# ratt-ru/pfb-clean

Hardware: AMD Instinct MI355X
Metric: PCG matvecs/sec (FFT-conv A^H A apply), 4k x 4k x 8-band cube (higher is better)
Workload: dtype f32; 1 GPU; 4096x4096x8-band cube PCG (hessian_psf + Tikhonov, M = x/sigmainv, tol=0, minit=maxit=20); nx_psf=8192, bands_per_gpu=8, parallelism=band-shard x1, allreduce_hook=False

## Files before the change

### include/pfb_hip.h

```cpp
#ifndef PFB_HIP_H
#define PFB_HIP_H

#include <stddef.h>
#include <stdint.h>

#ifdef __cplusplus
extern "C" {
#endif

#define PFB_ABI_VERSION 1

#define PFB_F32 0
#define PFB_F64 1

#define PFB_OK               0
#define PFB_ERR_INVALID     -1
#define PFB_ERR_UNSUPPORTED -2
#define PFB_ERR_HIP         -3
#define PFB_ERR_NONFINITE   -4
#define PFB_ERR_ALLOC       -5
#define PFB_ERR_COMM        -6

#define PFB_PCG_CONVERGED     0
#define PFB_PCG_MAXIT         1
#define PFB_PCG_ZERO_RESIDUAL 2
#define PFB_PCG_BREAKDOWN     3

int         pfb_abi_version(void);
const char* pfb_last_error(void);

typedef struct pfb_conv_plan pfb_conv_plan;

int pfb_psfconv_plan_create(int nx, int ny, int nx_psf, int ny_psf, int nband,
                            int dtype, pfb_conv_plan** plan);
int pfb_psfconv_plan_destroy(pfb_conv_plan* plan);

int pfb_psfconv_set_psfhat(pfb_conv_plan* plan, const void* psfhat, void* stream);

int pfb_psfconv_set_psf(pfb_conv_plan* plan, const void* psf, void* psfhat_out, void* stream);

int pfb_psfhat_from_psf(int dtype, const void* psf, int nband, int nx_psf, int ny_psf, void* psfhat, void* stream);

int pfb_psfhat_regrid(int dtype, const void* psfhat, int nband, int nx, int ny, int nx_psf, int ny_psf,
                      int nx_psf2, int ny_psf2, void* psfhat2, void* stream);

int pfb_psfconv_apply(pfb_conv_plan* plan, int band0, int nb,
                      const void* x, const void* beam, double wsum, double sigmainv,
                      void* out, const void* dot_with, double* dot_out, void* stream);

int pfb_psfconv_apply_dots(pfb_conv_plan* plan, int band0, int nb,
                           const void* x, const void* beam, double wsum, double sigmainv,
                           void* out, const void* dot_with, const void* dot_with2,
                           double* dots_out, void* stream);

int    pfb_psfconv_plan_info(const pfb_conv_plan* plan, int* fast_path, int* vb,
                             size_t* workspace_bytes);

int pfb_psfconv_set_profiling(pfb_conv_plan* plan, int on);
int pfb_psfconv_get_profile(pfb_conv_plan* plan, double stage_ms[3], int* napply);

#define PFB_REDUCE_WS_DOUBLES 8192

int pfb_dot(int dtype, const void* a, const void* b, size_t n,
            double* out, double* ws, void* stream);
int pfb_norm_diff_sums(int dtype, const void* x, const void* xp, size_t n,
                       double* out, double* ws, void* stream);
int pfb_any_nonzero(int dtype, const void* a, size_t n, double* out, double* ws,
                    void* stream);
int pfb_axpby(int dtype, double a, const void* x, double b, void* y, size_t n,
              void* stream);

typedef int (*pfb_allreduce_fn)(void* ctx, double* dev_buf, int count, void* stream);

typedef struct {
    int    status;
    int    iters;
    int    matvecs;
    int    backtracks;
    double eps;
    double rnorm;
} pfb_pcg_result;

size_t pfb_pcg_work_bytes(const pfb_conv_plan* plan, int nb);
int pfb_pcg_solve(pfb_conv_plan* plan, int band0, int nb,
                  const void* b, void* x, void* r_out,
                  const void* beam, double wsum, double sigmainv, double mdiv,
                  double tol, int maxit, int minit, int backtrack,
                  void* work, pfb_allreduce_fn allreduce, void* allreduce_ctx,
                  pfb_pcg_result* result, void* stream);
// ... 65 lines not shown
```

### pfb_clean_amd/_lib.py

```python
import ctypes as C
import os

_HERE = os.path.dirname(os.path.abspath(__file__))
LIB_PATH = os.environ.get('PFB_HIP_LIB') or os.path.join(_HERE, 'libpfb_hip.so')

PFB_F32, PFB_F64 = 0, 1
PFB_OK = 0
ERRORS = {-1: 'invalid argument', -2: 'unsupported size/dtype', -3: 'HIP runtime error',
          -4: 'non-finite value', -5: 'device allocation failed', -6: 'band-shard exchange failed'}
PCG_STATUS = {0: 'converged', 1: 'maxit', 2: 'zero-residual', 3: 'breakdown'}
REDUCE_WS_DOUBLES = 8192


PFB_ERR_INVALID = -1
PFB_ERR_UNSUPPORTED = -2
PFB_ERR_ALLOC = -5
PFB_ERR_COMM = -6


class PfbHipError(RuntimeError):
    def __init__(self, code, msg):
        super().__init__(f"libpfb_hip: {ERRORS.get(code, code)}: {msg}")
        self.code = code


class PfbCommError(PfbHipError):
    """PFB_ERR_COMM: the band-shard exchange of a distributed solve failed, was aborted or timed out.  The exchange has
    been torn down; this rank holds no result and should exit non-zero (its peers get the same error)."""


class PcgResult(C.Structure):
    _fields_ = [('status', C.c_int), ('iters', C.c_int), ('matvecs', C.c_int),
                ('backtracks', C.c_int), ('eps', C.c_double), ('rnorm', C.c_double)]


ALLREDUCE_FN = C.CFUNCTYPE(C.c_int, C.c_void_p, C.c_void_p, C.c_int, C.c_void_p)

_vp, _i, _d, _sz = C.c_void_p, C.c_int, C.c_double, C.c_size_t
SIGNATURES = {
    'pfb_abi_version': (_i, []),
    'pfb_last_error': (C.c_char_p, []),
    'pfb_psfconv_plan_create': (_i, [_i, _i, _i, _i, _i, _i, C.POINTER(_vp)]),
    'pfb_psfconv_plan_destroy': (_i, [_vp]),
    'pfb_psfconv_set_psfhat': (_i, [_vp, _vp, _vp]),
    'pfb_psfconv_apply': (_i, [_vp, _i, _i, _vp, _vp, _d, _d, _vp, _vp, _vp, _vp]),
    'pfb_psfconv_set_psf': (_i, [_vp, _vp, _vp, _vp]),
    'pfb_psfhat_regrid': (_i, [_i, _vp, _i, _i, _i, _i, _i, _i, _i, _vp, _vp]),
    'pfb_psfhat_from_psf': (_i, [_i, _vp, _i, _i, _i, _vp, _vp]),
    'pfb_psfconv_apply_dots': (_i, [_vp, _i, _i, _vp, _vp, _d, _d, _vp, _vp, _vp, _vp, _vp]),
    'pfb_psfconv_plan_info': (_i, [_vp, C.POINTER(_i), C.POINTER(_i), C.POINTER(_sz)]),
    'pfb_psfconv_set_profiling': (_i, [_vp, _i]),
    'pfb_psfconv_get_profile': (_i, [_vp, C.POINTER(_d), C.POINTER(_i)]),
    'pfb_dot': (_i, [_i, _vp, _vp, _sz, _vp, _vp, _vp]),
    'pfb_norm_diff_sums': (_i, [_i, _vp, _vp, _sz, _vp, _vp, _vp]),
    'pfb_any_nonzero': (_i, [_i, _vp, _sz, _vp, _vp, _vp]),
    'pfb_axpby': (_i, [_i, _d, _vp, _d, _vp, _sz, _vp]),
    'pfb_pcg_work_bytes': (_sz, [_vp, _i]),
    'pfb_pcg_solve': (_i, [_vp, _i, _i, _vp, _vp, _vp, _vp, _d, _d, _d, _d, _i, _i, _i,
                           _vp, ALLREDUCE_FN, _vp, C.POINTER(PcgResult), _vp]),
    'pfb_comm_bind': (_i, [C.c_char_p]),
    'pfb_comm_unique_id': (_i, [_vp]),
    'pfb_comm_init': (_i, [_i, _i, _vp, C.POINTER(_vp)]),
    'pfb_comm_destroy': (_i, [_vp]),
    'pfb_comm_info': (_i, [_vp, C.POINTER(_i), C.POINTER(_i), C.POINTER(_i), C.POINTER(_i)]),
    'pfb_comm_allreduce': (_i, [_vp, _vp, _i, _vp]),
    'pfb_comm_check': (_i, [_vp]),
    'pfb_comm_abort': (_i, [_vp]),
    'pfb_psi_plan_create': (_i, [_i, _i, _i, _i, C.POINTER(_i), C.POINTER(_d), _i, _i,
                                 C.POINTER(_vp)]),
    'pfb_psi_plan_destroy': (_i, [_vp]),
    'pfb_psi_plan_dims': (_i, [_vp, C.POINTER(_i), C.POINTER(_i)]),
    'pfb_psi_dot': (_i, [_vp, _vp, _vp, _vp]),
    'pfb_psi_hdot': (_i, [_vp, _vp, _vp, _vp]),
    'pfb_dual_update': (_i, [_i, _vp, _vp, _vp, _d, _d, _i, _sz, _vp, _vp]),
    'pfb_dual_bandsum': (_i, [_i, _vp, _vp, _d, _i, _sz, _vp, _vp]),
    'pfb_dual_apply': (_i, [_i, _vp, _vp, _vp, _vp, _d, _d, _i, _sz, _vp, _vp]),
    'pfb_prox_21': (_i, [_i, _vp, _vp, _vp, _d, _d, _i, _sz, _vp]),
    'pfb_dual_update_l2': (_i, [_i, _vp, _vp, _vp, _d, _d, _i, _sz, _vp]),
    'pfb_dual_bandsum_chunk': (_i, [_i, _vp, _vp, _d, _i, _sz, _sz, _vp, _vp]),
    'pfb_dual_apply_chunk': (_i, [_i, _vp, _vp, _vp, _vp, _d, _d, _i, _sz, _sz, _vp, _vp]),
    'pfb_clark_subminor': (_i, [_i, _vp, _sz, _i, _vp, _i, _i, _vp, _vp, _vp, _i, _i, _vp, _d, _d, _i, _vp, _vp]),
    'pfb_hogbom': (_i, [_i, _vp, _vp, _vp, _vp, _i, _i, _i, _i, _i, _d, _d, _d, _i, _vp, _sz, _vp, _vp, _vp]),
    'pfb_freqmul': (_i, [_i, _vp, _vp, _vp, _i, _sz, _vp, _vp, _vp]),
# ... 32 lines not shown
```

### pfb_clean_amd/csrc/cgvec.hip

```cpp
#include "conv_plan.hpp"
#include "pcg_state.hpp"
#include <chrono>
#include <unistd.h>
#include <cstring>
#include <cstdlib>

namespace pfb {

constexpr int RED_BLOCK = 256;
constexpr int RED_MAX_GRID = 1024;

static inline int red_grid(size_t nvec) {
    size_t g = (nvec + RED_BLOCK - 1) / RED_BLOCK;
    g = (g + 3) / 4;
    if (g < 1) g = 1;
    if (g > (size_t)RED_MAX_GRID) g = RED_MAX_GRID;
    return (int)g;
}

template <typename T> struct V16;
template <> struct V16<float>  { using type = float4;  static constexpr int N = 4; };
template <> struct V16<double> { using type = double2; static constexpr int N = 2; };

template <typename T, int V> struct Pack { T e[V]; };
// ... 523 lines not shown
    err = pfb_psfconv_apply(plan, band0, nb, xcur, beam, wsum, sigmainv, rcur, nullptr, nullptr, (void*)st);
    if (err != PFB_OK) return err;
    res->matvecs = 1;
    PFB_LAUNCH_VEC(T, k_pcg_init, n, (PL{rcur, b, p}), rcur, (const T*)b, p, mdiv);
    hipLaunchKernelGGL(k_final_sum, dim3(1), dim3(RED_BLOCK), 0, st, ws, G_used, 2, S + S_RHON);
    if ((err = reduce_hook(S_RHON, 2)) != PFB_OK) return err;
    hipLaunchKernelGGL(k_init_state, dim3(1), dim3(1), 0, st, S, tol, (double)minit, (double)maxit);
    if ((err = fetch()) != PFB_OK) return err;
    if (h[S_NUM] == 0.0) {
        res->status = PFB_PCG_ZERO_RESIDUAL;
        res->eps = 1.0;
        res->rnorm = h[S_RHO];
        if (r_out) PFB_HIP_CHECK(hipMemcpyAsync(r_out, rcur, n * sizeof(T), hipMemcpyDeviceToDevice, st));
        return wait_stream();
    }

    int k = 0;
    double eps = 1.0;
    double rho = h[S_RHO];
    int status = -1;
    if (backtrack != 1) {
        int khost = 0;
        bool pending_end = false;
        bool go = (1.0 > tol || 0 < minit) && 0 < maxit;
        bool lookahead = n <= ((size_t)4 << 20);
        if (const char* la = getenv("PFB_PCG_LOOKAHEAD")) lookahead = atoi(la) != 0;
        if (lookahead && !plan->pcg_pin) {
            PFB_HIP_CHECK(hipHostMalloc((void**)&plan->pcg_pin, sizeof(double) * 2 * S_NSCALAR, hipHostMallocDefault));
            PFB_HIP_CHECK(hipEventCreateWithFlags(&plan->pcg_ev[0], hipEventDisableTiming));
            PFB_HIP_CHECK(hipEventCreateWithFlags(&plan->pcg_ev[1], hipEventDisableTiming));
        }
        int slot = 0;
        bool have_prev = false, stale_h = false;
        while (go) {
            err = psfconv_apply_partials(plan, band0, nb, p, beam, wsum, sigmainv, Ap, p, rcur, (void*)st);
            if (err != PFB_OK) return err;
            const int predict = backtrack == 2 ? 2 : 3;
            hipLaunchKernelGGL(k_iter_sums, dim3(1), dim3(256), 0, st, (const double*)plan->partials,
                               plan->last_npartials, (const double*)ws, G_used, pending_end ? 1 : 0, S,
                               mdiv_d, predict, allreduce ? 0 : 1);
            if (allreduce) {
                if ((err = reduce_hook(S_PAP, pending_end ? 7 : 4)) != PFB_OK) return err;
                if (pending_end)
                    hipLaunchKernelGGL(k_iter_end_begin, dim3(1), dim3(1), 0, st, S, mdiv_d, predict);
                else
                    hipLaunchKernelGGL(k_iter_begin, dim3(1), dim3(1), 0, st, S, mdiv_d, predict);
            }
            pending_end = false;
            G_used = launch_update_dir<T>(n, xcur, rcur, p, Ap, xnew, rnew, S + S_ALPHA, mdiv, ws, st);
            if (khost + 1 < minit && khost + 1 < maxit) {
                pending_end = true;
            } else if (!allreduce) {
                hipLaunchKernelGGL(k_final_sum_waves_end, dim3(1), dim3(256), 0, st, ws, G_used, S);
            } else {
                hipLaunchKernelGGL(k_final_sum_waves, dim3(1), dim3(256), 0, st, ws, G_used, 4, S,
                                   (Dst4{{S_RHON, S_NUM, S_DEN, S_ANY}}));
                if ((err = reduce_hook(S_RHON, 3)) != PFB_OK) return err;
                hipLaunchKernelGGL(k_iter_end, dim3(1), dim3(1), 0, st, S, 1);
            }
            { T* t = xcur; xcur = xnew; xnew = t; t = rcur; rcur = rnew; rnew = t; }
            ++khost;
            if (khost < minit && khost < maxit) continue;
            if (lookahead && khost < maxit) {
                double* snap = plan->pcg_pin + (size_t)slot * S_NSCALAR;
                PFB_HIP_CHECK(hipMemcpyAsync(snap, S, sizeof(double) * S_NSCALAR, hipMemcpyDeviceToHost, st));
                PFB_HIP_CHECK(hipEventRecord(plan->pcg_ev[slot], st));
                stale_h = true;
                if (have_prev) {
                    if (allreduce) {
                        const auto t0 = std::chrono::steady_clock::now();
                        for (long spins = 0;; ++spins) {
                            const hipError_t q = hipEventQuery(plan->pcg_ev[slot ^ 1]);
                            if (q == hipSuccess) break;
                            if (q != hipErrorNotReady) { set_error("pcg: hipEventQuery -> %s", hipGetErrorString(q)); return PFB_ERR_HIP; }
                            if (spins < 4096) continue;
                            if (allreduce(actx, nullptr, 0, (void*)st) != 0) return comm_fail("the exchange reported a failure");
                            const double el = std::chrono::duration<double>(std::chrono::steady_clock::now() - t0).count();
                            if (el > comm_timeout) { set_error("%s", ""); return comm_fail("no progress on the solver's stream (PFB_COMM_TIMEOUT_S)"); }
                            usleep(el < 0.01 ? 20 : 500);
                        }
                    } else
// ... 141 lines not shown
```

### pfb_clean_amd/csrc/conv_plan.hpp

```cpp
#pragma once
#include "common.hpp"
#include "fft_generic.hpp"

struct pfb_conv_plan {
    int nx, ny, P, Q, M;
    int nband, dtype;
    int VB, nvb;
    int fast;
    int long_lines;
    void* long_ws;
    size_t long_ws_bytes;
    pfb::FftFactors frow;
    pfb::FftFactors fcol;
    void* twP;
    void* twQ;
    void* psf_l;
    void* T;
    double* partials;
    size_t T_elems_per_band;
    size_t psf_elems_per_band;
    size_t workspace_bytes;
    int have_psf;
    int partials_per_band;
    int last_npartials;
    void* fast_tables;
    int prof_on, prof_n, prof_tick;
    hipEvent_t* prof_ev;
    double* pcg_pin;
    hipEvent_t pcg_ev[2];
};

namespace pfb {
constexpr int PROF_MAX = 512;
inline void prof_mark(pfb_conv_plan* p, hipStream_t st, int k) {
    if (!p->prof_on) return;
    const bool sampled = (p->prof_tick % p->prof_on) == 0 && p->prof_n < PROF_MAX;
    if (sampled) (void)hipEventRecord(p->prof_ev[p->prof_n * 4 + k], st);
    if (k == 3) {
        if (sampled) p->prof_n++;
        p->prof_tick++;
    }
}
int psfconv_apply_partials(pfb_conv_plan* p, int band0, int nb, const void* x, const void* beam,
                           double wsum, double sigmainv, void* out, const void* dot_with,
                           const void* dot_with2, void* stream);
}
```

### pfb_clean_amd/csrc/fftconv.hip

```cpp
#include "conv_plan.hpp"
#include "fft_long.hpp"
#include <vector>
#include <cstring>
#include <cstdlib>

namespace pfb {

thread_local char g_err[512] = "";
void set_error(const char* fmt, ...) {
    va_list ap;
    va_start(ap, fmt);
    vsnprintf(g_err, sizeof(g_err), fmt, ap);
    va_end(ap);
}

bool pow2_supported(const pfb_conv_plan* p);
int pow2_apply(pfb_conv_plan* p, int band0, int nb, const void* x, const void* beam,
               double scale, double sigmainv, void* out, const void* dot_with, const void* dot_with2,
               hipStream_t st);
int pow2_prepare(pfb_conv_plan* p);
void pow2_release(pfb_conv_plan* p);
int pow2_rows_per_wg(const pfb_conv_plan* p);
int pow2_nblocks(const pfb_conv_plan* p);
int pow2_nvb(const pfb_conv_plan* p);
int pow2_set_psfhat(pfb_conv_plan* p, const void* psfhat, hipStream_t st);
int pow2_set_psf(pfb_conv_plan* p, const void* psf, void* psfhat_out, hipStream_t st);

struct ConvDims {
    int nx, ny, P, Q, M, VB, nvb;
    size_t T_band, psf_band;
};

__device__ __forceinline__ size_t t_index(const ConvDims& d, int band, int i, int v) {
    return (size_t)band * d.T_band + ((size_t)(v / d.VB) * d.nx + i) * d.VB + (v % d.VB);
}
__device__ __forceinline__ size_t psf_index(const ConvDims& d, int band, int u, int v) {
    return (size_t)band * d.psf_band + ((size_t)(v / d.VB) * d.P + u) * d.VB + (v % d.VB);
}

template <typename T>
__global__ void k_relayout_psfhat(const cplx<T>* __restrict__ psfhat, cplx<T>* __restrict__ psf_l,
                                  ConvDims d) {
    const int band = blockIdx.z;
    const int u = blockIdx.y;
    const int v = blockIdx.x * blockDim.x + threadIdx.x;
    if (v >= d.nvb * d.VB) return;
    cplx<T> val(0, 0);
    if (v <= d.M) val = psfhat[((size_t)band * d.P + u) * (d.M + 1) + v];
    psf_l[psf_index(d, band, u, v)] = val;
}

template <typename T>
// ... 412 lines not shown
    return PFB_OK;
}

int pfb_psfconv_plan_destroy(pfb_conv_plan* p) {
    if (!p) return PFB_OK;
    if (p->twP) (void)hipFree(p->twP);
    if (p->twQ) (void)hipFree(p->twQ);
    if (p->psf_l) (void)hipFree(p->psf_l);
    if (p->T) (void)hipFree(p->T);
    if (p->partials) (void)hipFree(p->partials);
    if (p->long_ws) (void)hipFree(p->long_ws);
    pow2_release(p);
    if (p->prof_ev) {
        for (int k = 0; k < 4 * PROF_MAX; ++k) (void)hipEventDestroy(p->prof_ev[k]);
        free(p->prof_ev);
    }
    if (p->pcg_pin) {
        (void)hipHostFree(p->pcg_pin);
        (void)hipEventDestroy(p->pcg_ev[0]);
        (void)hipEventDestroy(p->pcg_ev[1]);
    }
    free(p);
    return PFB_OK;
}

int pfb_psfconv_plan_info(const pfb_conv_plan* p, int* fast_path, int* vb, size_t* workspace_bytes) {
    PFB_REQUIRE(p != nullptr, PFB_ERR_INVALID, "plan_info: null plan");
    if (fast_path) *fast_path = p->fast;
    if (vb) *vb = p->VB;
    if (workspace_bytes) *workspace_bytes = p->workspace_bytes;
    return PFB_OK;
}

int pfb_psfconv_set_profiling(pfb_conv_plan* p, int on) {
    PFB_REQUIRE(p != nullptr, PFB_ERR_INVALID, "set_profiling: null plan");
    if (on && !p->prof_ev) {
        p->prof_ev = (hipEvent_t*)calloc(4 * PROF_MAX, sizeof(hipEvent_t));
        PFB_REQUIRE(p->prof_ev != nullptr, PFB_ERR_ALLOC, "set_profiling: host alloc failed");
        for (int k = 0; k < 4 * PROF_MAX; ++k) PFB_HIP_CHECK(hipEventCreate(&p->prof_ev[k]));
    }
    p->prof_on = on > 0 ? on : 0;
    p->prof_n = 0;
    p->prof_tick = 0;
    return PFB_OK;
}

int pfb_psfconv_get_profile(pfb_conv_plan* p, double* stage_ms, int* napply) {
    PFB_REQUIRE(p && stage_ms && napply, PFB_ERR_INVALID, "get_profile: null argument");
    stage_ms[0] = stage_ms[1] = stage_ms[2] = 0.0;
    *napply = p->prof_n;
    for (int a = 0; a < p->prof_n; ++a) {
        PFB_HIP_CHECK(hipEventSynchronize(p->prof_ev[a * 4 + 3]));
        for (int k = 0; k < 3; ++k) {
            float ms = 0.f;
            PFB_HIP_CHECK(hipEventElapsedTime(&ms, p->prof_ev[a * 4 + k], p->prof_ev[a * 4 + k + 1]));
            stage_ms[k] += ms;
        }
    }
    p->prof_n = 0;
    return PFB_OK;
}

int pfb_psfconv_set_psfhat(pfb_conv_plan* p, const void* psfhat, void* stream) {
    PFB_REQUIRE(p && psfhat, PFB_ERR_INVALID, "set_psfhat: null argument");
    if (p->fast) {
        int rc = pow2_set_psfhat(p, psfhat, as_stream(stream));
// ... 31 lines not shown
    int rc = p->dtype == PFB_F32
        ? psfhat_from_psf_t<float>(psf, dst, p->nband, p->P, p->Q, p->frow, p->fcol, p->twP, p->twQ, st)
        : psfhat_from_psf_t<double>(psf, dst, p->nband, p->P, p->Q, p->frow, p->fcol, p->twP, p->twQ, st);
    if (rc == PFB_OK) rc = pfb_psfconv_set_psfhat(p, dst, stream);
    if (tmp) {
        (void)hipStreamSynchronize(st);
        (void)hipFree(tmp);
    }
    return rc;
}

int pfb_psfhat_from_psf(int dtype, const void* psf, int nband, int nx_psf, int ny_psf, void* psfhat, void* stream) {
    PFB_REQUIRE(psf && psfhat && nband > 0 && nx_psf > 0 && ny_psf > 0, PFB_ERR_INVALID, "psfhat_from_psf: bad argument");
    PFB_REQUIRE(dtype == PFB_F32 || dtype == PFB_F64, PFB_ERR_INVALID, "psfhat_from_psf: bad dtype");
    PFB_REQUIRE(ny_psf % 2 == 0, PFB_ERR_UNSUPPORTED, "psfhat_from_psf: ny_psf=%d must be even", ny_psf);
    return dtype == PFB_F32 ? psfhat_from_psf_grid<float>(psf, psfhat, nband, nx_psf, ny_psf, as_stream(stream))
                            : psfhat_from_psf_grid<double>(psf, psfhat, nband, nx_psf, ny_psf, as_stream(stream));
}

int pfb_psfhat_regrid(int dtype, const void* psfhat, int nband, int nx, int ny, int nx_psf, int ny_psf,
                      int nx_psf2, int ny_psf2, void* psfhat2, void* stream) {
    PFB_REQUIRE(psfhat && psfhat2 && nband > 0 && nx > 0 && ny > 0, PFB_ERR_INVALID, "psfhat_regrid: bad argument");
    PFB_REQUIRE(dtype == PFB_F32 || dtype == PFB_F64, PFB_ERR_INVALID, "psfhat_regrid: bad dtype");
    PFB_REQUIRE(ny_psf % 2 == 0 && ny_psf2 % 2 == 0, PFB_ERR_UNSUPPORTED, "psfhat_regrid: odd last axis");
    PFB_REQUIRE(nx_psf2 >= 2 * nx - 1 && ny_psf2 >= 2 * ny - 1, PFB_ERR_INVALID,
                "psfhat_regrid: the new grid (%d,%d) must hold every offset of a (%d,%d) image", nx_psf2, ny_psf2, nx, ny);
    return dtype == PFB_F32
        ? psfhat_regrid_t<float>(psfhat, nband, nx, ny, nx_psf, ny_psf, nx_psf2, ny_psf2, psfhat2, as_stream(stream))
        : psfhat_regrid_t<double>(psfhat, nband, nx, ny, nx_psf, ny_psf, nx_psf2, ny_psf2, psfhat2, as_stream(stream));
}

static int apply_common(pfb_conv_plan* p, int band0, int nb, const void* x, const void* beam,
                        double wsum, double sigmainv, void* out, const void* dot_with,
                        const void* dot_with2, double* dots_out, int ndots, void* stream) {
    PFB_REQUIRE(p && x && out, PFB_ERR_INVALID, "apply: null argument");
    PFB_REQUIRE(p->have_psf, PFB_ERR_INVALID, "apply: pfb_psfconv_set_psfhat was never called");
    PFB_REQUIRE(band0 >= 0 && nb > 0 && band0 + nb <= p->nband, PFB_ERR_INVALID,
                "apply: band range [%d,%d) outside plan (nband=%d)", band0, band0 + nb, p->nband);
    PFB_REQUIRE(x != out, PFB_ERR_INVALID, "apply: out must not alias x");
    PFB_REQUIRE(!dot_with || dots_out || ndots == 0, PFB_ERR_INVALID, "apply: dot_with given without an output");
    PFB_REQUIRE(!dot_with2 || dot_with, PFB_ERR_INVALID, "apply: dot_with2 needs dot_with");
    hipStream_t st = as_stream(stream);
    double scale = 1.0 / ((double)p->P * (double)p->Q);
    if (wsum > 0) scale /= wsum;
    int rc;
    p->last_npartials = p->partials_per_band * nb;
    if (p->fast)
        rc = pow2_apply(p, band0, nb, x, beam, scale, sigmainv, out, dot_with, dot_with2, st);
    else if (p->long_lines) {
        const size_t need = p->dtype == PFB_F32 ? long_apply_ws_bytes<float>(nb, p->nx, p->M, p->P)
                                                : long_apply_ws_bytes<double>(nb, p->nx, p->M, p->P);
        if (need > p->long_ws_bytes) {
            PFB_HIP_CHECK(hipStreamSynchronize(st));
            if (p->long_ws) (void)hipFree(p->long_ws);
            p->long_ws = nullptr; p->long_ws_bytes = 0;
            if (hipMalloc(&p->long_ws, need) != hipSuccess) {
                set_error("apply: workspace allocation of %zu B for the long-line path failed", need);
                return PFB_ERR_ALLOC;
            }
            p->long_ws_bytes = need;
        }
        prof_mark(p, st, 0); prof_mark(p, st, 1); prof_mark(p, st, 2);
        if (p->dtype == PFB_F32)
            rc = apply_long<float>((cplx<float>*)p->long_ws, (cplx<float>*)p->T, (const cplx<float>*)p->psf_l, p->partials,
                                   (const cplx<float>*)p->twP, (const cplx<float>*)p->twQ, p->frow, p->fcol, p->nx, p->ny,
                                   p->P, p->M, p->T_elems_per_band, p->psf_elems_per_band, band0, nb, (const float*)x,
                                   (const float*)beam, scale, sigmainv, (float*)out, (const float*)dot_with,
                                   (const float*)dot_with2, st);
        else
            rc = apply_long<double>((cplx<double>*)p->long_ws, (cplx<double>*)p->T, (const cplx<double>*)p->psf_l,
                                    p->partials, (const cplx<double>*)p->twP, (const cplx<double>*)p->twQ, p->frow, p->fcol,
                                    p->nx, p->ny, p->P, p->M, p->T_elems_per_band, p->psf_elems_per_band, band0, nb,
                                    (const double*)x, (const double*)beam, scale, sigmainv, (double*)out,
                                    (const double*)dot_with, (const double*)dot_with2, st);
        prof_mark(p, st, 3);
    } else if (p->dtype == PFB_F32)
        rc = apply_generic<float>(p, band0, nb, x, beam, scale, sigmainv, out, dot_with, dot_with2, st);
    else
        rc = apply_generic<double>(p, band0, nb, x, beam, scale, sigmainv, out, dot_with, dot_with2, st);
    if (rc != PFB_OK) return rc;
    if (dot_with && ndots > 0) {
        hipLaunchKernelGGL(k_sum_partials, dim3(1), dim3(256), 0, st, p->partials,
                           p->last_npartials, ndots, dots_out);
        PFB_HIP_CHECK(hipGetLastError());
    }
    return PFB_OK;
}

int pfb_psfconv_apply(pfb_conv_plan* p, int band0, int nb, const void* x, const void* beam,
                      double wsum, double sigmainv, void* out, const void* dot_with,
                      double* dot_out, void* stream) {
    return apply_common(p, band0, nb, x, beam, wsum, sigmainv, out, dot_with, nullptr, dot_out, 1, stream);
}

int pfb_psfconv_apply_dots(pfb_conv_plan* p, int band0, int nb, const void* x, const void* beam,
                           double wsum, double sigmainv, void* out, const void* dot_with,
                           const void* dot_with2, double* dots_out, void* stream) {
    PFB_REQUIRE(dot_with && dots_out, PFB_ERR_INVALID, "apply_dots: dot_with and dots_out are required");
    return apply_common(p, band0, nb, x, beam, wsum, sigmainv, out, dot_with, dot_with2, dots_out, 3, stream);
}

}

int pfb::psfconv_apply_partials(pfb_conv_plan* p, int band0, int nb, const void* x, const void* beam,
                                double wsum, double sigmainv, void* out, const void* dot_with,
                                const void* dot_with2, void* stream) {
    PFB_REQUIRE(dot_with, PFB_ERR_INVALID, "apply_partials: dot_with is required");
    return apply_common(p, band0, nb, x, beam, wsum, sigmainv, out, dot_with, dot_with2, nullptr, 0, stream);
}
```

### pfb_clean_amd/csrc/fftconv_pow2.hip

```cpp
#include "conv_plan.hpp"
#include "fft_pow2.hpp"
#include <vector>
#include <cstdlib>

#ifndef PFB_POW2_PART
#define PFB_POW2_PART 0
#endif
#define PFB_POW2_COL  (PFB_POW2_PART != 1)
#define PFB_POW2_REST (PFB_POW2_PART != 2)

namespace pfb {

#ifndef PFB_STAMP
#define PFB_STAMP 0
#endif
#if PFB_STAMP
#define PFB_STAMP_ITS 4
#define PFB_STAMP_FIRST 2
static __device__ unsigned long long* g_stamp_buf = nullptr;
#define STAMP(KID, it, slot)                                                                              \
    do {                                                                                                  \
        const unsigned _si = (unsigned)((it) - PFB_STAMP_FIRST);                                          \
        if (threadIdx.x == 0 && g_stamp_buf && _si < PFB_STAMP_ITS && blockIdx.x < 1024)                  \
            g_stamp_buf[(((size_t)(KID) * 1024 + blockIdx.x) * PFB_STAMP_ITS + _si) * 16 + (slot)] = wall_clock64(); \
    } while (0)
#else
#define STAMP(KID, it, slot) do { (void)(it); } while (0)
#endif

template <typename T> struct FastCfg;
template <> struct FastCfg<float>  { static constexpr int ECOL = 8; static constexpr int EROWMAX = 32; static constexpr int WCOL = 4; static constexpr int NVB = 2; };
template <> struct FastCfg<double> { static constexpr int ECOL = 8; static constexpr int EROWMAX = 16; static constexpr int WCOL = 2; static constexpr int NVB = 1; };

template <typename T, int L, int E, int GMAX> constexpr int row_groups();
// ... 952 lines not shown
            for (int j = 0; j < E; ++j) {
                vv[j] = cplx<T>(xa[j].x, xa[j].y) * P::tw_row(ltm, t, j);
                if ((j & 3) == 3) __builtin_amdgcn_sched_barrier(0);
            }
            const int bln = vbn / tiles_per_band, i0n = P::tile_row(vbn - bln * tiles_per_band, tiles_per_band);
            const size_t offn = (size_t)bln * d.xband + (size_t)(i0n + g) * d.xpitch;
            const V2* xr = reinterpret_cast<const V2*>(x + offn) + t;
            const V2* br = BEAM ? reinterpret_cast<const V2*>(beam + offn) + t : nullptr;
            F::template run<false>(vv, lds, t, ltw, [&](auto k) {
                constexpr int K = decltype(k)::value;
#pragma unroll
                for (int j = (K * E) / NP; j < ((K + 1) * E) / NP; ++j) {
                    xa[j] = xr[TPB * j];
                    if constexpr (BEAM) ba[j] = br[TPB * j];
                }
            });
            STAMP(0, sit, 5);
        }
        {
            const int tid = launder((int)threadIdx.x);
            const int g = tid / TPB, t = tid % TPB;
            cplx<T>* wp = lds0 + (size_t)g * P::STRIDE + F::pad(t);
            __syncthreads();
#pragma unroll
            for (int j = 0; j < E; ++j) wp[F::cpad(TPB * j)] = vv[j];
            __syncthreads();
            fwdp_post<T, L, 1>(lds0 + (size_t)(tid % G) * P::STRIDE, ltm, wq1, Tb, d.nx, i0, tid % G, tid / G);
            STAMP(0, sit, 6);
            __syncthreads();
        }
        STAMP(0, sit, 7);
        if (vbn == vb) break;
        vb = vbn;
    }
}

template <typename T, int L, int E, int PAR, typename PF>
__device__ __forceinline__ void row_inv_phase(PF&& after_loads_issued, const cplx<T>* __restrict__ Tb,
                                              const cplx<T>* __restrict__ twQ,
                                              const cplx<T>* __restrict__ ptw, cplx<T>* lds0,
                                              cplx<T>* lds, int nx, int i0, int t,
                                              cplx<T> (&vv)[E]) {
    using F = RegFft<T, L, E, RowCfg<T, L, true>::WAVE, InvDb<T, L>::OFF, true>;
    constexpr int TPB = F::TPB;
    constexpr int G = row_groups<T, L, E, RowCfg<T, L, true>::GMAX>();
    constexpr int NT = G * TPB;
    constexpr int STRIDE = F::LDS_ELEMS + 4;
    const int rr = threadIdx.x % G, bi = threadIdx.x / G;
    cplx<T>* yr = lds0 + (size_t)rr * STRIDE;
    __syncthreads();
    constexpr int NVB = FastCfg<T>::NVB;
    constexpr int NBE = (L + NVB) / NVB;
    constexpr int NBP = PAR ? L / NVB : NBE;
    constexpr int BSTEP = NT / G;
    const cplx<T>* Tp = Tb + ((size_t)(PAR ? NBE : 0) * nx + i0 + rr) * NVB;
    constexpr int NIT = (NBP + BSTEP - 1) / BSTEP;
    Blk<T, NVB> y[NIT];
#pragma unroll
    for (int k = 0; k < NIT; ++k) {
        const int b = bi + k * BSTEP;
        if (b < NBP) y[k] = loadb<T, NVB>(Tp + (size_t)b * nx * NVB);
    }
    after_loads_issued();
#pragma unroll
    for (int k = 0; k < NIT; ++k) {
        const int b = bi + k * BSTEP;
// ... 543 lines not shown
template <typename T, int N, int E>
static int prep_ptw_compact(void** dev) {
    constexpr int n = ptw_total<N, E>() / 4;
    std::vector<cplx<T>> h(n > 0 ? n : 1);
    if (n > 0) fill_ptw_compact<T, N, E>(h.data());
    PFB_HIP_CHECK(hipMalloc(dev, sizeof(cplx<T>) * h.size()));
    PFB_HIP_CHECK(hipMemcpy(*dev, h.data(), sizeof(cplx<T>) * h.size(), hipMemcpyHostToDevice));
    return PFB_OK;
}

template <typename T, int L>
static int set_invp_attr() {
    constexpr int E = InvPE<T, L>::E;
    if constexpr (InvP<T, L, E>::OK) {
#define PFB_INVATTR(MODE, BM)                                                                           \
        PFB_HIP_CHECK(hipFuncSetAttribute((const void*)(k_row_inv_pow2p<T, L, E, MODE, BM>),             \
                                          hipFuncAttributeMaxDynamicSharedMemorySize, 160 * 1024))
        PFB_INVATTR(0, false); PFB_INVATTR(1, false); PFB_INVATTR(2, false);
        PFB_INVATTR(0, true);  PFB_INVATTR(1, true);  PFB_INVATTR(2, true);
#undef PFB_INVATTR
    }
    return PFB_OK;
}

template <typename T, int L>
static int prep_fwdp(void** table) {
    if constexpr (FwdP<T, L>::OK) {
        int rc = prep_ptw_compact<T, L, FwdP<T, L>::EOK>(table);
        if (rc != PFB_OK) return rc;
        PFB_HIP_CHECK(hipFuncSetAttribute((const void*)(k_row_fwd_pow2q<T, L, false>),
                                          hipFuncAttributeMaxDynamicSharedMemorySize, 160 * 1024));
        PFB_HIP_CHECK(hipFuncSetAttribute((const void*)(k_row_fwd_pow2q<T, L, true>),
                                          hipFuncAttributeMaxDynamicSharedMemorySize, 160 * 1024));
    } else {
        PFB_HIP_CHECK(hipFuncSetAttribute((const void*)k_row_fwd_pow2<T, L, RowCfg<T, L, false>::E>,
                                          hipFuncAttributeMaxDynamicSharedMemorySize, 160 * 1024));
    }
    return PFB_OK;
}


template <typename T>
static int prep_tables(pfb_conv_plan* p, FastTables* ft) {
    const int H = p->nx, L = p->ny / 2;
    int rc = PFB_ERR_UNSUPPORTED;
    constexpr int lds_max = 160 * 1024;
    switch (H) {
#define X(NN) case NN: rc = prep_ptw<T, NN, ecol<T, NN>()>(&ft->ptw_col);                          \
        if (rc == PFB_OK) rc = prep_ptw_compact<T, NN, ecol<T, NN>()>(&ft->ptwc_col);             \
        if (rc == PFB_OK && NN == 8192) rc = prep_ptw_compact<T, 4096, ECOLX>(&ft->ptwc_col_x);         \
        if (rc == PFB_OK) rc = pow2_col_set_attr(p->dtype, NN); break;
        PFB_POW2_SIZES(X)
#undef X
        default: break;
    }
    if (rc != PFB_OK) return rc;
    rc = PFB_ERR_UNSUPPORTED;
    switch (L) {
#define X(NN) case NN: rc = prep_ptw<T, NN, RowCfg<T, NN, false>::E>(&ft->ptw_row);                   \
        if (rc == PFB_OK) rc = prep_ptw_compact<T, NN, RowCfg<T, NN, true>::E>(&ft->ptw_row_inv);    \
        if (rc == PFB_OK) { if (InvPE<T, NN>::E != RowCfg<T, NN, true>::E) rc = prep_ptw_compact<T, NN, InvPE<T, NN>::E>(&ft->ptw_row_inv_p); \
                            else ft->ptw_row_inv_p = ft->ptw_row_inv; }                            \
        if (rc == PFB_OK) PFB_HIP_CHECK(hipFuncSetAttribute((const void*)k_row_inv_pow2<T, NN, RowCfg<T, NN, true>::E>, \
            hipFuncAttributeMaxDynamicSharedMemorySize, lds_max));                                   \
        if (rc == PFB_OK) rc = set_invp_attr<T, NN>();                                               \
        if (rc == PFB_OK) rc = prep_fwdp<T, NN>(&ft->ptwc_row_fwd); break;
// ... 258 lines not shown
    return PFB_OK;
}
int pow2_col_fwd_launch(pfb_conv_plan* p, const FastTables* ft, const void* Tq, int band, hipStream_t st) {
    return p->dtype == PFB_F32 ? col_fwd_launch_t<float>(p, ft, Tq, band, st) : col_fwd_launch_t<double>(p, ft, Tq, band, st);
}
#endif

#if PFB_POW2_REST

template <typename T, int L>
static void launch_row_fwd(pfb_conv_plan* p, const FastTables* ft, void* Tbuf, int band0, int nb, const void* x,
                           const void* beam, size_t xpitch, size_t xband, hipStream_t st) {
    FastDims d{p->nx, p->ny, p->M, p->T_elems_per_band, p->psf_elems_per_band, xpitch, xband};
    if constexpr (FwdP<T, L>::OK) {
        using FP = FwdP<T, L>;
        const int tiles_per_band = p->nx / FP::G, ntiles = tiles_per_band * nb;
        const int grid = ntiles < ft->num_cu * FP::WG_PER_CU ? ntiles : ft->num_cu * FP::WG_PER_CU;
        const long double a = 6.283185307179586476925286766559005768L / (2.0L * (long double)p->ny);
        const cplx<T> wq1((T)cosl(a), (T)(-sinl(a)));
#define PFB_FWDQ(BM)                                                                                              \
        hipLaunchKernelGGL((k_row_fwd_pow2q<T, L, BM>), dim3(grid), dim3(FP::NT), FP::LDS, st, (const T*)x,      \
                           (const T*)beam, (cplx<T>*)Tbuf, (const cplx<T>*)ft->twM,                              \
                           (const cplx<T>*)ft->ptwc_row_fwd, d, band0, tiles_per_band, ntiles, wq1)
        if (beam) PFB_FWDQ(true); else PFB_FWDQ(false);
#undef PFB_FWDQ
    } else {
        constexpr int E = RowCfg<T, L, false>::E;
        using F = RegFft<T, L, E, RowCfg<T, L, false>::WAVE>;
        constexpr int G = row_groups<T, L, E, RowCfg<T, L, false>::GMAX>();
        const size_t lds = sizeof(cplx<T>) * (size_t)G * (F::LDS_ELEMS + 4);
        hipLaunchKernelGGL((k_row_fwd_pow2<T, L, E>), dim3(p->nx / G, nb), dim3(G * F::TPB), lds, st,
                           (const T*)x, (const T*)beam, (cplx<T>*)Tbuf, (const cplx<T>*)p->twQ,
                           (const cplx<T>*)ft->twM, (const cplx<T>*)ft->ptw_row, d, band0);
    }
}

template <typename T, int L>
static void launch_row_inv(pfb_conv_plan* p, const FastTables* ft, int band0, int nb, const void* x,
                           const void* beam, double scale, double sigmainv, void* out,
                           const void* dot_with, const void* dot_with2, hipStream_t st) {
    constexpr int E = RowCfg<T, L, true>::E;
    using F = RegFft<T, L, E, RowCfg<T, L, true>::WAVE>;
    constexpr int G = row_groups<T, L, E, RowCfg<T, L, true>::GMAX>();
    FastDims d{p->nx, p->ny, p->M, p->T_elems_per_band, p->psf_elems_per_band, (size_t)p->ny, (size_t)p->nx * p->ny};
    constexpr int EP = InvPE<T, L>::E;
    if constexpr (InvP<T, L, EP>::OK) {
        const bool plain_dots = !dot_with || (dot_with == x);
        if (plain_dots && !(dot_with2 && !dot_with)) {
            using IP = InvP<T, L, EP>;
            const int tiles_per_band = p->nx / IP::G, ntiles = tiles_per_band * nb;
            const int grid = ntiles < IP::WG_PER_CU * ft->num_cu ? ntiles : IP::WG_PER_CU * ft->num_cu;
            const long double a = 6.283185307179586476925286766559005768L / (2.0L * (long double)p->ny);
            const cplx<T> wq1((T)cosl(a), (T)(-sinl(a)));
#define PFB_INVP2(MODE, BM)                                                                             \
            hipLaunchKernelGGL((k_row_inv_pow2p<T, L, EP, MODE, BM>), dim3(grid), dim3(IP::NT), IP::LDS, st, \
                               (const cplx<T>*)p->T, (const cplx<T>*)ft->twM,                           \
                               (const cplx<T>*)ft->ptw_row_inv_p, (const T*)x, (const T*)beam,          \
                               (const T*)dot_with2, (T*)out, p->partials, d, band0, tiles_per_band,     \
                               ntiles, (T)scale, (T)sigmainv, wq1)
#define PFB_INVP(MODE) do { if (beam) PFB_INVP2(MODE, true); else PFB_INVP2(MODE, false); } while (0)
            p->last_npartials = grid;
            if (!dot_with) PFB_INVP(0);
            else if (!dot_with2) PFB_INVP(1);
            else PFB_INVP(2);
#undef PFB_INVP
#undef PFB_INVP2
            return;
        }
    }
    const size_t lds = 384 + sizeof(cplx<T>) * ((size_t)((F::PTWC + 1) & ~1) + (size_t)G * (F::LDS_ELEMS + 4) * (InvDb<T, L>::ON ? 2 : 1));
    hipLaunchKernelGGL((k_row_inv_pow2<T, L, E>), dim3(p->nx / G, nb), dim3(G * F::TPB), lds, st,
                       (const cplx<T>*)p->T, (const cplx<T>*)p->twQ, (const cplx<T>*)ft->twM,
                       (const cplx<T>*)ft->ptw_row_inv, (const T*)x, (const T*)beam, (const T*)dot_with,
                       (const T*)dot_with2, (T*)out, p->partials, d, band0, (T)scale, (T)sigmainv);
}

template <typename T>
static int apply_t(pfb_conv_plan* p, int band0, int nb, const void* x, const void* beam, double scale,
                   double sigmainv, void* out, const void* dot_with, const void* dot_with2, hipStream_t st) {
    const FastTables* ft = (const FastTables*)p->fast_tables;
    const int H = p->nx, L = p->ny / 2;
    prof_mark(p, st, 0);
    switch (L) {
#define X(NN) case NN: launch_row_fwd<T, NN>(p, ft, p->T, band0, nb, x, beam, (size_t)p->ny, (size_t)p->nx * p->ny, st); break;
        PFB_POW2_SIZES(X)
#undef X
        default: set_error("pow2_apply: unsupported ny"); return PFB_ERR_UNSUPPORTED;
    }
    prof_mark(p, st, 1);
    if (int rc = pow2_col_launch(p, ft, band0, nb, st); rc != PFB_OK) return rc;
    prof_mark(p, st, 2);
    switch (L) {
#define X(NN) case NN: launch_row_inv<T, NN>(p, ft, band0, nb, x, beam, scale, sigmainv, out, dot_with, dot_with2, st); break;
        PFB_POW2_SIZES(X)
#undef X
        default: break;
    }
    prof_mark(p, st, 3);
    PFB_HIP_CHECK(hipGetLastError());
    return PFB_OK;
}

int pow2_apply(pfb_conv_plan* p, int band0, int nb, const void* x, const void* beam, double scale,
               double sigmainv, void* out, const void* dot_with, const void* dot_with2, hipStream_t st) {
    return p->dtype == PFB_F32 ? apply_t<float>(p, band0, nb, x, beam, scale, sigmainv, out, dot_with, dot_with2, st)
                               : apply_t<double>(p, band0, nb, x, beam, scale, sigmainv, out, dot_with, dot_with2, st);
}
#endif

}

#if PFB_STAMP && PFB_POW2_REST
extern "C" int pfb_debug_set_stamps(void* buf) { return pfb::pow2_set_stamp((unsigned long long*)buf); }
#endif
```

Measured before the change: 435.2 cube-matvecs/s.

## Fuse PCG x/r/p update into forward row-FFT kernel of next matvec

Result: faster. 441.9 cube-matvecs/s, median of 6 (+1.5%).

```diff
diff --git a/include/pfb_hip.h b/include/pfb_hip.h
--- a/include/pfb_hip.h
+++ b/include/pfb_hip.h
@@ -55,6 +55,7 @@
 
 int    pfb_psfconv_plan_info(const pfb_conv_plan* plan, int* fast_path, int* vb,
                              size_t* workspace_bytes);
+int    pfb_pcg_fused_update(const pfb_conv_plan* plan, int nb, int with_beam);
 
 int pfb_psfconv_set_profiling(pfb_conv_plan* plan, int on);
 int pfb_psfconv_get_profile(pfb_conv_plan* plan, double stage_ms[3], int* napply);
diff --git a/pfb_clean_amd/_lib.py b/pfb_clean_amd/_lib.py
--- a/pfb_clean_amd/_lib.py
+++ b/pfb_clean_amd/_lib.py
@@ -49,6 +49,7 @@
     'pfb_psfhat_from_psf': (_i, [_i, _vp, _i, _i, _i, _vp, _vp]),
     'pfb_psfconv_apply_dots': (_i, [_vp, _i, _i, _vp, _vp, _d, _d, _vp, _vp, _vp, _vp, _vp]),
     'pfb_psfconv_plan_info': (_i, [_vp, C.POINTER(_i), C.POINTER(_i), C.POINTER(_sz)]),
+    'pfb_pcg_fused_update': (_i, [_vp, _i, _i]),
     'pfb_psfconv_set_profiling': (_i, [_vp, _i]),
     'pfb_psfconv_get_profile': (_i, [_vp, C.POINTER(_d), C.POINTER(_i)]),
     'pfb_dot': (_i, [_i, _vp, _vp, _sz, _vp, _vp, _vp]),
diff --git a/pfb_clean_amd/csrc/cgvec.hip b/pfb_clean_amd/csrc/cgvec.hip
--- a/pfb_clean_amd/csrc/cgvec.hip
+++ b/pfb_clean_amd/csrc/cgvec.hip
@@ -579,9 +579,20 @@
         }
         int slot = 0;
         bool have_prev = false, stale_h = false;
+        const bool fuse_upd = psfconv_fused_update_ok(plan, nb, beam) && can_vec<T>(n, PL{x, r, p, Ap, xalt, ralt});
+        bool upd_in_conv = false;
         while (go) {
-            err = psfconv_apply_partials(plan, band0, nb, p, beam, wsum, sigmainv, Ap, p, rcur, (void*)st);
-            if (err != PFB_OK) return err;
+            if (upd_in_conv) {
+                PcgUpdate u{xcur, rcur, p, Ap, xnew, rnew, S + S_ALPHA, (double)mdiv, ws, 0};
+                err = psfconv_apply_update_partials(plan, band0, nb, &u, wsum, sigmainv, Ap, rnew, (void*)st);
+                if (err != PFB_OK) return err;
+                G_used = u.grid;
+                { T* t = xcur; xcur = xnew; xnew = t; t = rcur; rcur = rnew; rnew = t; }
+                upd_in_conv = false;
+            } else {
+                err = psfconv_apply_partials(plan, band0, nb, p, beam, wsum, sigmainv, Ap, p, rcur, (void*)st);
+                if (err != PFB_OK) return err;
+            }
             const int predict = backtrack == 2 ? 2 : 3;
             hipLaunchKernelGGL(k_iter_sums, dim3(1), dim3(256), 0, st, (const double*)plan->partials,
                                plan->last_npartials, (const double*)ws, G_used, pending_end ? 1 : 0, S,
@@ -594,6 +605,12 @@
                     hipLaunchKernelGGL(k_iter_begin, dim3(1), dim3(1), 0, st, S, mdiv_d, predict);
             }
             pending_end = false;
+            if (khost + 1 < minit && khost + 1 < maxit && fuse_upd) {
+                upd_in_conv = true;
+                pending_end = true;
+                ++khost;
+                continue;
+            }
             G_used = launch_update_dir<T>(n, xcur, rcur, p, Ap, xnew, rnew, S + S_ALPHA, mdiv, ws, st);
             if (khost + 1 < minit && khost + 1 < maxit) {
                 pending_end = true;
diff --git a/pfb_clean_amd/csrc/conv_plan.hpp b/pfb_clean_amd/csrc/conv_plan.hpp
--- a/pfb_clean_amd/csrc/conv_plan.hpp
+++ b/pfb_clean_amd/csrc/conv_plan.hpp
@@ -41,6 +41,16 @@
         p->prof_tick++;
     }
 }
+struct PcgUpdate {
+    const void* x; const void* r; void* p; const void* Ap; void* xn; void* rn;
+    const double* S_alpha;
+    double mdiv;
+    double* ws;
+    int grid;
+};
+bool psfconv_fused_update_ok(const pfb_conv_plan* p, int nb, const void* beam);
+int psfconv_apply_update_partials(pfb_conv_plan* p, int band0, int nb, PcgUpdate* upd, double wsum, double sigmainv,
+                                  void* out, const void* dot_with2, void* stream);
 int psfconv_apply_partials(pfb_conv_plan* p, int band0, int nb, const void* x, const void* beam,
                            double wsum, double sigmainv, void* out, const void* dot_with,
                            const void* dot_with2, void* stream);
diff --git a/pfb_clean_amd/csrc/fftconv.hip b/pfb_clean_amd/csrc/fftconv.hip
--- a/pfb_clean_amd/csrc/fftconv.hip
+++ b/pfb_clean_amd/csrc/fftconv.hip
@@ -17,7 +17,8 @@
 bool pow2_supported(const pfb_conv_plan* p);
 int pow2_apply(pfb_conv_plan* p, int band0, int nb, const void* x, const void* beam,
                double scale, double sigmainv, void* out, const void* dot_with, const void* dot_with2,
-               hipStream_t st);
+               PcgUpdate* upd, hipStream_t st);
+bool pow2_fused_update_ok(const pfb_conv_plan* p);
 int pow2_prepare(pfb_conv_plan* p);
 void pow2_release(pfb_conv_plan* p);
 int pow2_rows_per_wg(const pfb_conv_plan* p);
@@ -496,6 +497,11 @@
     return PFB_OK;
 }
 
+int pfb_pcg_fused_update(const pfb_conv_plan* p, int nb, int with_beam) {
+    PFB_REQUIRE(p != nullptr, PFB_ERR_INVALID, "pcg_fused_update: null plan");
+    return psfconv_fused_update_ok(p, nb, with_beam ? p : nullptr) ? 1 : 0;
+}
+
 int pfb_psfconv_set_profiling(pfb_conv_plan* p, int on) {
     PFB_REQUIRE(p != nullptr, PFB_ERR_INVALID, "set_profiling: null plan");
     if (on && !p->prof_ev) {
@@ -593,7 +599,8 @@
 
 static int apply_common(pfb_conv_plan* p, int band0, int nb, const void* x, const void* beam,
                         double wsum, double sigmainv, void* out, const void* dot_with,
-                        const void* dot_with2, double* dots_out, int ndots, void* stream) {
+                        const void* dot_with2, double* dots_out, int ndots, void* stream,
+                        PcgUpdate* upd = nullptr) {
     PFB_REQUIRE(p && x && out, PFB_ERR_INVALID, "apply: null argument");
     PFB_REQUIRE(p->have_psf, PFB_ERR_INVALID, "apply: pfb_psfconv_set_psfhat was never called");
     PFB_REQUIRE(band0 >= 0 && nb > 0 && band0 + nb <= p->nband, PFB_ERR_INVALID,
@@ -607,8 +614,11 @@
     int rc;
     p->last_npartials = p->partials_per_band * nb;
     if (p->fast)
-        rc = pow2_apply(p, band0, nb, x, beam, scale, sigmainv, out, dot_with, dot_with2, st);
-    else if (p->long_lines) {
+        rc = pow2_apply(p, band0, nb, x, beam, scale, sigmainv, out, dot_with, dot_with2, upd, st);
+    else if (upd) {
+        set_error("apply: the fused PCG update needs the pow2 path");
+        return PFB_ERR_UNSUPPORTED;
+    } else if (p->long_lines) {
         const size_t need = p->dtype == PFB_F32 ? long_apply_ws_bytes<float>(nb, p->nx, p->M, p->P)
                                                 : long_apply_ws_bytes<double>(nb, p->nx, p->M, p->P);
         if (need > p->long_ws_bytes) {
@@ -669,3 +679,15 @@
     PFB_REQUIRE(dot_with, PFB_ERR_INVALID, "apply_partials: dot_with is required");
     return apply_common(p, band0, nb, x, beam, wsum, sigmainv, out, dot_with, dot_with2, nullptr, 0, stream);
 }
+
+bool pfb::psfconv_fused_update_ok(const pfb_conv_plan* p, int nb, const void* beam) {
+    (void)nb;
+    return p && p->fast && !beam && pow2_fused_update_ok(p);
+}
+
+int pfb::psfconv_apply_update_partials(pfb_conv_plan* p, int band0, int nb, PcgUpdate* upd, double wsum,
+                                       double sigmainv, void* out, const void* dot_with2, void* stream) {
+    PFB_REQUIRE(upd && psfconv_fused_update_ok(p, nb, nullptr), PFB_ERR_UNSUPPORTED,
+                "apply_update_partials: no fused update kernel for this plan");
+    return apply_common(p, band0, nb, upd->p, nullptr, wsum, sigmainv, out, upd->p, dot_with2, nullptr, 0, stream, upd);
+}
diff --git a/pfb_clean_amd/csrc/fftconv_pow2.hip b/pfb_clean_amd/csrc/fftconv_pow2.hip
--- a/pfb_clean_amd/csrc/fftconv_pow2.hip
+++ b/pfb_clean_amd/csrc/fftconv_pow2.hip
@@ -1,5 +1,6 @@
 #include "conv_plan.hpp"
 #include "fft_pow2.hpp"
+#include "pcg_state.hpp"
 #include <vector>
 #include <cstdlib>
 
@@ -1018,6 +1019,208 @@
         STAMP(0, sit, 7);
         if (vbn == vb) break;
         vb = vbn;
+    }
+}
+
+template <typename T>
+struct UpdArgs {
+    const T* x; const T* r; T* p; const T* Ap; T* xn; T* rn;
+    const double* S_alpha;
+    T mdiv;
+    double* ws;
+};
+template <typename T, int L>
+struct FwdU {
+    using P = FwdP<T, L>;
+    static constexpr int NW = P::NT / 64;
+    static constexpr size_t LDS = P::LDS + sizeof(double) * 4 * NW;
+    static constexpr bool OK = P::OK && sizeof(T) == 4 && L == 2048 && LDS <= (size_t)160 * 1024;
+};
+template <typename T, int L>
+__global__ void __launch_bounds__((FwdP<T, L>::NT))
+k_row_fwd_upd_pow2q(UpdArgs<T> u, cplx<T>* __restrict__ Tw, const cplx<T>* __restrict__ twM,
+                    const cplx<T>* __restrict__ ptwc, FastDims d, int band0, int tiles_per_band, int ntiles,
+                    cplx<T> wq1) {
+    using P = FwdP<T, L>;
+    constexpr int E = P::EOK;
+    using F = RegFft<T, L, E, false, 0, true, false>;
+    constexpr int TPB = F::TPB, G = P::G, NT = P::NT, NP = F::NPASS, NW = FwdU<T, L>::NW;
+    using V2 = typename vec2<T>::type;
+    extern __shared__ __attribute__((aligned(16))) char smem[];
+    cplx<T>* ltw = reinterpret_cast<cplx<T>*>(smem);
+    cplx<T>* ltm = ltw + P::PTWP;
+    cplx<T>* lds0 = ltm + P::NTM;
+    double* lacc = reinterpret_cast<double*>(lds0 + (size_t)G * P::STRIDE);
+    const bool dead = u.S_alpha[S_DEAD - S_ALPHA] != 0.0 || u.S_alpha[S_STOP - S_ALPHA] != 0.0;
+    const T alpha = dead ? T(0) : (T)u.S_alpha[0];
+    const T beta = (T)u.S_alpha[S_BETA - S_ALPHA];
+    const T mdiv = u.mdiv;
+    int vb = blockIdx.x;
+    if (vb >= ntiles) {
+        if (threadIdx.x < 4) u.ws[(size_t)threadIdx.x * gridDim.x + blockIdx.x] = 0.0;
+        return;
+    }
+    for (int k = threadIdx.x; k < F::PTWC; k += NT) ltw[k] = ptwc[k];
+    for (int k = threadIdx.x; k < P::NTM; k += NT) ltm[k] = twM[k];
+    for (int k = threadIdx.x; k < 4 * NW; k += NT) lacc[k] = 0.0;
+    auto add_sum = [&](int q, double v) {
+        v = wave_sum(v);
+        if ((threadIdx.x & 63) == 0) lacc[q * NW + (threadIdx.x >> 6)] += v;
+    };
+    auto tile_off = [&](int tile, int g) -> size_t {
+        const int bl = tile / tiles_per_band, i0 = P::tile_row(tile - bl * tiles_per_band, tiles_per_band);
+        return (size_t)bl * d.xband + (size_t)(i0 + g) * d.xpitch;
+    };
+    V2 A[E], B[E], C[E];
+    auto form_r = [&](auto j0, auto j1, V2* rw, const V2* pr) {
+#pragma unroll
+        for (int j = decltype(j0)::value; j < decltype(j1)::value; ++j) {
+            A[j].x = A[j].x + alpha * B[j].x;
+            A[j].y = A[j].y + alpha * B[j].y;
+            rw[TPB * j] = A[j];
+        }
+#pragma unroll
+        for (int j = decltype(j0)::value; j < decltype(j1)::value; ++j) B[j] = pr[TPB * j];
+    };
+    using J0 = std::integral_constant<int, 0>;
+    using JH = std::integral_constant<int, E / 2>;
+    using JE = std::integral_constant<int, E>;
+    {
+        const int g = threadIdx.x / TPB, t = threadIdx.x % TPB;
+        const size_t off = tile_off(vb, g);
+        const V2* rr = reinterpret_cast<const V2*>(u.r + off) + t;
+        const V2* qr = reinterpret_cast<const V2*>(u.Ap + off) + t;
+#pragma unroll
+        for (int j = 0; j < E; ++j) { A[j] = rr[TPB * j]; B[j] = qr[TPB * j]; }
+        form_r(J0{}, JE{}, reinterpret_cast<V2*>(u.rn + off) + t, reinterpret_cast<const V2*>(u.p + off) + t);
+    }
+    __syncthreads();
+    for (int sit = 0;; ++sit) {
+        const int vbn = vb + (int)gridDim.x < ntiles ? vb + (int)gridDim.x : vb;
+        const int bl = vb / tiles_per_band, i0 = P::tile_row(vb - bl * tiles_per_band, tiles_per_band);
+        cplx<T>* Tb = Tw + (size_t)(band0 + bl) * d.T_band;
+        cplx<T> vv[E];
+        {
+            const int tid = launder((int)threadIdx.x);
+            const int g = tid / TPB, t = tid % TPB;
+            V2* pw = reinterpret_cast<V2*>(u.p + tile_off(vb, g)) + t;
+            const T dv = mdiv > T(0) ? mdiv : T(1);
+            const T be = dead ? T(1) : beta, ym = dead ? T(0) : T(1);
+            double s0 = 0.0;
+            int s3 = 0;
+#pragma unroll
+            for (int j = 0; j < E; ++j) {
+                const T yx = A[j].x / dv, yy = A[j].y / dv;
+                s0 += (double)A[j].x * (double)yx;
+                s0 += (double)A[j].y * (double)yy;
+                V2 pn;
+                pn.x = fma(be, B[j].x, -(yx * ym));
+                pn.y = fma(be, B[j].y, -(yy * ym));
+                s3 += (pn.x != T(0) ? 1 : 0) + (pn.y != T(0) ? 1 : 0);
+                pw[TPB * j] = pn;
+                vv[j] = cplx<T>(pn.x, pn.y);
+                C[j] = B[j];
+            }
+            add_sum(0, s0);
+            add_sum(3, (double)s3);
+        }
+        {
+            const int tid = launder((int)threadIdx.x);
+            const int g = tid / TPB, t = tid % TPB;
+            cplx<T>* lds = lds0 + (size_t)g * P::STRIDE;
+            const V2* xr = reinterpret_cast<const V2*>(u.x + tile_off(vb, g)) + t;
+            F::template run<false>(vv, lds, t, ltw, [&](auto k) {
+                constexpr int K = decltype(k)::value;
+#pragma unroll
+                for (int j = (K * E) / NP; j < ((K + 1) * E) / NP; ++j) A[j] = xr[TPB * j];
+            });
+        }
+        {
+            const int tid = launder((int)threadIdx.x);
+            const int g = tid / TPB, t = tid % TPB;
+            __syncthreads();
+            cplx<T>* wp = lds0 + (size_t)g * P::STRIDE + F::pad(t);
+#pragma unroll
+            for (int j = 0; j < E; ++j) wp[F::cpad(TPB * j)] = vv[j];
+            __syncthreads();
+        }
+        {
+            const int tid = launder((int)threadIdx.x);
+            const int g = tid / TPB, t = tid % TPB;
+            V2* xw = reinterpret_cast<V2*>(u.xn + tile_off(vb, g)) + t;
+            double s1 = 0.0, s2 = 0.0;
+#pragma unroll
+            for (int j = 0; j < E; ++j) {
+                V2 xv;
+                xv.x = A[j].x + alpha * C[j].x;
+                xv.y = A[j].y + alpha * C[j].y;
+                const double dx = (double)xv.x - (double)A[j].x, dy = (double)xv.y - (double)A[j].y;
+                s1 += dx * dx;
+                s2 += (double)xv.x * (double)xv.x;
+                s1 += dy * dy;
+                s2 += (double)xv.y * (double)xv.y;
+                xw[TPB * j] = xv;
+            }
+            add_sum(1, s1);
+            add_sum(2, s2);
+        }
+        {
+            const int tid = launder((int)threadIdx.x);
+            const int g = tid / TPB, t = tid % TPB;
+            const V2* pr = opaque(reinterpret_cast<const V2*>(u.p + tile_off(vb, g)) + t);
+            const V2* rr = reinterpret_cast<const V2*>(u.r + tile_off(vbn, g)) + t;
+            fwdp_post<T, L, 0>(lds0 + (size_t)(tid % G) * P::STRIDE, ltm, wq1, Tb, d.nx, i0, tid % G, tid / G,
+                               [&](auto k) {
+                                   if constexpr (decltype(k)::value == 0) {
+#pragma unroll
+                                       for (int j = 0; j < E; ++j) B[j] = pr[TPB * j];
+#pragma unroll
+                                       for (int j = 0; j < E; ++j) A[j] = rr[TPB * j];
+                                   }
+                               });
+        }
+        {
+            const int tid = launder((int)threadIdx.x);
+            const int g = tid / TPB, t = tid % TPB;
+            cplx<T>* lds = lds0 + (size_t)g * P::STRIDE;
+#pragma unroll
+            for (int j = 0; j < E; ++j) {
+                vv[j] = cplx<T>(B[j].x, B[j].y) * P::tw_row(ltm, t, j);
+                if ((j & 3) == 3) __builtin_amdgcn_sched_barrier(0);
+            }
+            const V2* qr = reinterpret_cast<const V2*>(u.Ap + tile_off(vbn, g)) + t;
+            F::template run<false>(vv, lds, t, ltw, [&](auto k) {
+                constexpr int K = decltype(k)::value;
+#pragma unroll
+                for (int j = (K * E) / NP; j < ((K + 1) * E) / NP; ++j) B[j] = qr[TPB * j];
+            });
+        }
+        {
+            const int tid = launder((int)threadIdx.x);
+            const int g = tid / TPB, t = tid % TPB;
+            cplx<T>* wp = lds0 + (size_t)g * P::STRIDE + F::pad(t);
+            const size_t offn = tile_off(vbn, g);
+            V2* rw = reinterpret_cast<V2*>(u.rn + offn) + t;
+            const V2* pr = reinterpret_cast<const V2*>(u.p + offn) + t;
+            __syncthreads();
+#pragma unroll
+            for (int j = 0; j < E; ++j) wp[F::cpad(TPB * j)] = vv[j];
+            __syncthreads();
+            fwdp_post<T, L, 1>(lds0 + (size_t)(tid % G) * P::STRIDE, ltm, wq1, Tb, d.nx, i0, tid % G, tid / G,
+                               [&](auto k) {
+                                   constexpr int K = decltype(k)::value;
+                                   if constexpr (K == 0) form_r(J0{}, JH{}, rw, pr);
+                                   if constexpr (K == 1) form_r(JH{}, JE{}, rw, pr);
+                               });
+            __syncthreads();
+        }
+        if (vbn == vb) break;
+        vb = vbn;
+    }
+    if (threadIdx.x < 4) {
+        double s = 0.0;
+        for (int w = 0; w < NW; ++w) s += lacc[threadIdx.x * NW + w];
+        u.ws[(size_t)threadIdx.x * gridDim.x + blockIdx.x] = s;
     }
 }
 
@@ -1627,6 +1830,9 @@
                                           hipFuncAttributeMaxDynamicSharedMemorySize, 160 * 1024));
         PFB_HIP_CHECK(hipFuncSetAttribute((const void*)(k_row_fwd_pow2q<T, L, true>),
                                           hipFuncAttributeMaxDynamicSharedMemorySize, 160 * 1024));
+        if constexpr (FwdU<T, L>::OK)
+            PFB_HIP_CHECK(hipFuncSetAttribute((const void*)(k_row_fwd_upd_pow2q<T, L>),
+                                              hipFuncAttributeMaxDynamicSharedMemorySize, 160 * 1024));
     } else {
         PFB_HIP_CHECK(hipFuncSetAttribute((const void*)k_row_fwd_pow2<T, L, RowCfg<T, L, false>::E>,
                                           hipFuncAttributeMaxDynamicSharedMemorySize, 160 * 1024));
@@ -1951,6 +2157,36 @@
         hipLaunchKernelGGL((k_row_fwd_pow2<T, L, E>), dim3(p->nx / G, nb), dim3(G * F::TPB), lds, st,
                            (const T*)x, (const T*)beam, (cplx<T>*)Tbuf, (const cplx<T>*)p->twQ,
                            (const cplx<T>*)ft->twM, (const cplx<T>*)ft->ptw_row, d, band0);
+    }
+}
+
+template <typename T, int L>
+static int launch_row_fwd_upd(pfb_conv_plan* p, const FastTables* ft, int band0, int nb, const PcgUpdate* pu,
+                              hipStream_t st) {
+    if constexpr (FwdU<T, L>::OK) {
+        using FP = FwdP<T, L>;
+        FastDims d{p->nx, p->ny, p->M, p->T_elems_per_band, p->psf_elems_per_band, (size_t)p->ny, (size_t)p->nx * p->ny};
+        const int tiles_per_band = p->nx / FP::G, ntiles = tiles_per_band * nb;
+        const int grid = ntiles < ft->num_cu * FP::WG_PER_CU ? ntiles : ft->num_cu * FP::WG_PER_CU;
+        const long double a = 6.283185307179586476925286766559005768L / (2.0L * (long double)p->ny);
+        const cplx<T> wq1((T)cosl(a), (T)(-sinl(a)));
+        const UpdArgs<T> u{(const T*)pu->x, (const T*)pu->r, (T*)pu->p, (const T*)pu->Ap, (T*)pu->xn, (T*)pu->rn,
+                           pu->S_alpha, (T)pu->mdiv, pu->ws};
+        constexpr size_t lds = FwdU<T, L>::LDS;
+        hipLaunchKernelGGL((k_row_fwd_upd_pow2q<T, L>), dim3(grid), dim3(FP::NT), lds, st, u, (cplx<T>*)p->T,
+                           (const cplx<T>*)ft->twM, (const cplx<T>*)ft->ptwc_row_fwd, d, band0, tiles_per_band, ntiles, wq1);
+        return grid;
+    }
+    return -1;
+}
+
+bool pow2_fused_update_ok(const pfb_conv_plan* p) {
+    if (p->dtype != PFB_F32) return false;
+    switch (p->ny / 2) {
+#define X(NN) case NN: return FwdU<float, NN>::OK;
+        PFB_POW2_SIZES(X)
+#undef X
+        default: return false;
     }
 }
 
@@ -1996,15 +2232,28 @@
 
 template <typename T>
 static int apply_t(pfb_conv_plan* p, int band0, int nb, const void* x, const void* beam, double scale,
-                   double sigmainv, void* out, const void* dot_with, const void* dot_with2, hipStream_t st) {
+                   double sigmainv, void* out, const void* dot_with, const void* dot_with2, PcgUpdate* upd,
+                   hipStream_t st) {
     const FastTables* ft = (const FastTables*)p->fast_tables;
     const int H = p->nx, L = p->ny / 2;
     prof_mark(p, st, 0);
-    switch (L) {
+    if (upd) {
+        int g = -1;
+        switch (L) {
+#define X(NN) case NN: g = launch_row_fwd_upd<T, NN>(p, ft, band0, nb, upd, st); break;
+            PFB_POW2_SIZES(X)
+#undef X
+            default: break;
+        }
+        PFB_REQUIRE(g > 0, PFB_ERR_UNSUPPORTED, "pow2_apply: no fused update kernel for ny = %d", p->ny);
+        upd->grid = g;
+    } else {
+        switch (L) {
 #define X(NN) case NN: launch_row_fwd<T, NN>(p, ft, p->T, band0, nb, x, beam, (size_t)p->ny, (size_t)p->nx * p->ny, st); break;
-        PFB_POW2_SIZES(X)
+            PFB_POW2_SIZES(X)
 #undef X
-        default: set_error("pow2_apply: unsupported ny"); return PFB_ERR_UNSUPPORTED;
+            default: set_error("pow2_apply: unsupported ny"); return PFB_ERR_UNSUPPORTED;
+        }
     }
     prof_mark(p, st, 1);
     if (int rc = pow2_col_launch(p, ft, band0, nb, st); rc != PFB_OK) return rc;
@@ -2021,9 +2270,9 @@
 }
 
 int pow2_apply(pfb_conv_plan* p, int band0, int nb, const void* x, const void* beam, double scale,
-               double sigmainv, void* out, const void* dot_with, const void* dot_with2, hipStream_t st) {
-    return p->dtype == PFB_F32 ? apply_t<float>(p, band0, nb, x, beam, scale, sigmainv, out, dot_with, dot_with2, st)
-                               : apply_t<double>(p, band0, nb, x, beam, scale, sigmainv, out, dot_with, dot_with2, st);
+               double sigmainv, void* out, const void* dot_with, const void* dot_with2, PcgUpdate* upd, hipStream_t st) {
+    return p->dtype == PFB_F32 ? apply_t<float>(p, band0, nb, x, beam, scale, sigmainv, out, dot_with, dot_with2, upd, st)
+                               : apply_t<double>(p, band0, nb, x, beam, scale, sigmainv, out, dot_with, dot_with2, upd, st);
 }
 #endif
 
```
